# sirpkt/flink-tensorflow

Hardware: AMD Instinct MI355X
Metric: records/sec (whole node) + p50 per-record latency, ResNet-50 stream DP=1/8 (higher is better)
Workload: dtype bf16

## Files before the change

### flink_tensorflow_amd/config.py

```python
from __future__ import annotations

import argparse
import contextlib
import dataclasses
import os
from dataclasses import dataclass, field
from typing import Any

_HBM_BYTES_MI355X = 288 * 1024 ** 3


@dataclass
class EngineConfig:
    parallelism: int = 1
    max_batch: int = 256
    max_delay_ms: float = 10.0
    precision: str = "bf16"
    batch_buckets: tuple = (64, 256)
    arena_fraction: float = 0.9
    use_hip_graph: bool = True
    pipeline_depth: int = 3
    checkpoint_interval_s: float | None = None
    checkpoint_dir: str | None = None
    restart_attempts: int = 0
    restart_delay_s: float = 0.0
    channel_capacity: int = 1024
    log_level: str = "INFO"
    sibling_conv_fusion: bool = True
    fuse_preprocess_stem: bool = True
    fuse_block_tails: bool = True
    decimate_tails: bool = True
    recompute_tails: bool = True
    chain_max_links: int = 2
    pw_res_kernel: bool = True
    conv3x3c64_kernel: bool = True
    chain_batch: int = -1
    chain_min_hw: int = 5041
    chain_edge: bool = True
    wd_fused_step: bool = True
    wd_sparse_exchange: str = "owner"
    wd_bucket_slack: float = 2.0
    jpeg_decode: str = "host"
    extra: dict = field(default_factory=dict)

    @classmethod
    def field_names(cls) -> list[str]:
        return [f.name for f in dataclasses.fields(cls) if f.name != "extra"]

    def _coerce(self, name: str, value: Any) -> Any:
        cur = getattr(self, name)
        typ = {f.name: f.type for f in dataclasses.fields(self)}[name]
        if value is None:
            return None
        if isinstance(value, str):
            if "tuple" in str(typ):
                return tuple(int(v) for v in value.replace(" ", "").split(",") if v)
            if "bool" in str(typ):
                return value.lower() in ("1", "true", "yes", "on")
            if "int" in str(typ) and "float" not in str(typ):
                return int(value)
            if "float" in str(typ):
                return float(value)
            return value
        if isinstance(cur, tuple) and isinstance(value, (list, tuple)):
            return tuple(value)
        return value

    def update(self, values: dict) -> "EngineConfig":
        for k, v in values.items():
            if k in self.field_names():
                setattr(self, k, self._coerce(k, v))
            else:
                self.extra[k] = v
        self.validate()
        return self

    @classmethod
    def from_yaml(cls, path: str, base: "EngineConfig | None" = None) -> "EngineConfig":
        import yaml

        with open(path) as f:
            data = yaml.safe_load(f) or {}
        return (base or cls()).update(data)

    @classmethod
    def from_env(cls, base: "EngineConfig | None" = None, prefix: str = "FT_", environ=None) -> "EngineConfig":
        environ = os.environ if environ is None else environ
        vals = {}
        for name in cls.field_names():
            key = prefix + name.upper()
            if key in environ:
                vals[name] = environ[key]
        return (base or cls()).update(vals)

    @classmethod
    def add_arguments(cls, ap: argparse.ArgumentParser) -> None:
        for name in cls.field_names():
            ap.add_argument("--" + name.replace("_", "-"), dest=f"cfg_{name}", default=None)
        ap.add_argument("--config", dest="cfg_yaml", default=None, help="YAML engine config")

    @classmethod
    def load(cls, argv: list[str] | None = None, environ=None) -> "EngineConfig":
        ap = argparse.ArgumentParser(add_help=False)
        cls.add_arguments(ap)
        ns, _ = ap.parse_known_args(argv if argv is not None else [])
        environ = os.environ if environ is None else environ
        cfg = cls()
        yml = ns.cfg_yaml or environ.get("FT_CONFIG")
        if yml:
            cfg = cls.from_yaml(yml, cfg)
        cfg = cls.from_env(cfg, environ=environ)
        cli = {n: getattr(ns, f"cfg_{n}") for n in cls.field_names() if getattr(ns, f"cfg_{n}") is not None}
        return cfg.update(cli)

    def validate(self) -> None:
        if self.parallelism < 1:
            raise ValueError("parallelism must be >= 1")
        if self.max_batch < 1 or self.max_delay_ms < 0:
# ... 73 lines not shown
```

### flink_tensorflow_amd/graph/conv_lowering.py

```python
from __future__ import annotations

from dataclasses import dataclass

import numpy as np
import torch

from ..ops import fp8 as F8
from ..ops import kernels as K
from ..types.names import TensorName
from .graph import Node
from .ops_nn import same_pads
from .plan import CompileError, Val, _cfg, _coff, _eff_scale, _root, _target, _view

_ACTS = {"Relu": K.ACT_RELU, "Relu6": K.ACT_RELU6, "Sigmoid": K.ACT_SIGMOID, "Tanh": K.ACT_TANH}

LITE_FP8_CFG = 11
_PP_MIN_K = 512

_PLAIN_ACTS = (K.ACT_NONE, K.ACT_RELU)
_DW_ACTS = {"Relu": K.ACT_RELU, "Relu6": K.ACT_RELU6}


@dataclass(frozen=True)
class ConvSite:
# ... 217 lines not shown
            w = w * scale
        w_dev = self._dev(w.reshape(KH * KW, C).contiguous(), torch.bfloat16)
        b_dev = self._dev(bias, torch.float32) if bias is not None else None
        self.params += [w_dev] + ([b_dev] if b_dev is not None else [])
        xin = self._as_bf16(x, node.name)
        out = self._new((N, Ho, Wo, C))
        for a in absorbed:
            self._fused.add(a.name)

        def run(xin=xin, out=out, w_dev=w_dev, b_dev=b_dev):
            K.dwconv2d_nhwc(xin.buf, w_dev, b_dev, stride, pads, dil, act, out=_target(out),
                            out_channel_offset=_coff(out), kernel=(KH, KW))

        self._emit(node.name, "dwconv", run, [xin], [out], {"impl": K.dwconv_impl(KH, KW, stride, dil)})
        self._finish_conv(last, absorbed, out)

    def _prepare_conv(self, node, x, w, bias, residual, act, last, absorbed, stride, pads, dil, out_hw,
                      cout_logical: int | None = None) -> _ConvJob:
        KH, KW, Cin, Cout = w.shape
        padded = cout_logical is not None and cout_logical != Cout
        N, H, W, C = x.shape
        s2d = self._s2d_ok(x, node, C, *stride, *dil, pads[0], pads[2], H, W)
        if s2d:
            w_ohwi, pads = K.s2d_stem_weights(w, H, W, pads)
            x.pre_cfg["s2d"] = True
            x.buf_shape = (N, (H + 1) // 2, (W + 1) // 2, 16)
            x.phys_c = 16
            stride = (1, 1)
            cin_pad = 16
        else:
            phys = x.phys_c or C
            cin_pad = -(-phys // 8) * 8
            w_ohwi = w.permute(3, 0, 1, 2).contiguous()
            if cin_pad != Cin:
                w_ohwi = torch.nn.functional.pad(w_ohwi, (0, cin_pad - Cin))
        w_dev = self._dev(w_ohwi, torch.bfloat16)
        b_dev = self._dev(bias, torch.float32) if bias is not None else None
        self.params += [w_dev] + ([b_dev] if b_dev is not None else [])
        out = self._new((N, *out_hw, cout_logical if padded else Cout), phys_c=Cout if padded else None)
        kernel = tuple(w_ohwi.shape[1:3])
        if (not padded and self.precision == "fp8" and residual is None and act in _PLAIN_ACTS and Cout % 16 == 0
                and self._fp8_consumers_ok(last.name) and self._qscale(last.name) is not None
                and _dconv_ok(self.device.type == "cuda", cin_pad, kernel, stride, dil, 2, False, act)):
            out = self._new((N, *out_hw, Cout), torch.uint8)
            out.qscale = self._qscale(last.name)
        res_val = add_node = None
        if residual is not None:
            add_node, ri = residual
            res_val = self.vals[add_node.inputs[ri]]
        xin = x if s2d else self._ensure_padded(x, cin_pad, node.name)
        for a in absorbed:
            self._fused.add(a.name)
        cfg = _cfg()
        site = ConvSite(
            on_gpu=self.device.type == "cuda", x_shape=tuple(xin.shape), cin=Cin, cin_phys=xin.phys_c or Cin, cout=Cout,
            kernel=kernel, stride=tuple(stride), pads=tuple(pads), dil=tuple(dil), act=act,
            residual=res_val is not None,
            res_plain=(res_val is not None and res_val.qscale is None and res_val.concat_slot is None
                       and tuple(res_val.shape) == tuple(out.shape)),
            res_alias=res_val is not None and res_val.alias_of is not None,
            x_dtype=xin.dtype, out_dtype=out.dtype, out_fp8=out.qscale is not None, out_coff=_coff(out), s2d=s2d,
            conv3x3c64_kernel=cfg.conv3x3c64_kernel, pw_res_kernel=cfg.pw_res_kernel)
        return _ConvJob(node, site, x, xin, out, res_val, add_node, w_ohwi, bias, w_dev, b_dev, last, absorbed)

    def _zero_bias(self, c: _ConvJob) -> torch.Tensor:
        return c.b_dev if c.b_dev is not None else self._dev(torch.zeros(c.site.cout), torch.float32)

    def _emit_dconv(self, c: _ConvJob):
        s, out = c.site, c.out
        Cout, conv_out = s.cout, tuple(c.out.shape)
        bn = 64 if Cout >= 64 else 32
        w_arr = self._dev(K.dconv_bf16_weight_bytes(c.w_ohwi, bn))
        b_dev = c.b_dev if c.b_dev is not None else torch.zeros(Cout, dtype=torch.float32, device=self.device)
        self.params += [w_arr, b_dev]
        pool = self._fusable_maxpool(c.last, s.act, out)
        mpad = None
        if pool is not None:
            pnode, mpad, (Hp, Wp) = pool
            out = self._new((conv_out[0], Hp, Wp, Cout))
            self._fused.add(pnode.name)
        elif self._fold_preprocess(c, w_arr, b_dev, bn):
            return

        def run_d(xin=c.xin, out=out, w_arr=w_arr, b_dev=b_dev, bn=bn, mpad=mpad):
            K.conv2d_direct(xin.buf, w_arr, s.kernel, Cout, b_dev, s.stride, s.pads, s.act,
                            out=_target(out), out_channel_offset=_coff(out), bn=bn,
                            out_scale=_eff_scale(out) if out.qscale is not None else None, maxpool_pad=mpad)

        self._emit(c.node.name, "conv", run_d, [c.xin], [out], {"conv_out": conv_out} if pool else None)
        if pool is not None:
            self.vals[(pool[0].name, 0)] = out
            self.stats["fused_pools"] += 1
            return
        self._finish_conv(c.last, c.absorbed, out)

    def _fold_preprocess(self, c: _ConvJob, w_arr, b_dev, bn) -> bool:
        s, x, out = c.site, c.x, c.out
        pp = x.pre_params
        if not (s.s2d and pp is not None and not pp["resize"]
                and _cfg().fuse_preprocess_stem and len(self.steps) == 1 and self.steps[0].kind == "preprocess"
                and self.steps[0].outputs[0] is x and _root(out) is out and _coff(out) == 0):
            return False
        self.steps.pop()
        xu = pp["x"]
        osc = _eff_scale(out) if out.qscale is not None else None

        def run_u(x=xu, out=out, w_arr=w_arr, b_dev=b_dev, bn=bn, osc=osc, mean=pp["mean"], std=pp["std"],
                  pads=s.pads):
            K.conv2d_direct_u8s2d(x.buf, w_arr, s.kernel, s.cout, b_dev, pads, s.act, mean, std, out=out.buf,
                                  bn=bn, out_scale=osc)

        self._emit(c.node.name, "preprocess", run_u, [xu], [out],
                   {"impl": "dconv_u8s2d", "conv_out": tuple(out.shape)})
        self.stats["fused_preprocess"] = 1
        self._finish_conv(c.last, c.absorbed, out)
        return True

    def _emit_conv3x3c64(self, c: _ConvJob):
        bz, act = self._zero_bias(c), c.site.act

        def run_c(xin=c.xin, out=c.out, w_dev=c.w_dev, bz=bz):
            K.conv3x3_c64(xin.buf, w_dev, bz, act, out=_target(out), out_channel_offset=_coff(out))

        self._emit(c.node.name, "conv", run_c, [c.xin], [c.out], {"impl": "conv3x3c64"})
        self.stats["conv3x3c64"] += 1
        self._finish_conv(c.last, c.absorbed, c.out)

    def _emit_gemm_pp(self, c: _ConvJob):
        Cin, Cout = c.site.cin, c.site.cout
        w_nk = c.w_dev.reshape(Cout, Cin)
        bz = self._zero_bias(c)
        M = int(np.prod(c.xin.shape[:-1]))
        splits = K.gemm_pp_splits(M, Cout, Cin)
        ws = torch.empty(splits * M * Cout, dtype=torch.float32, device=self.device) if splits > 1 else None

        def run_pp(xin=c.xin, out=c.out, w_nk=w_nk, bz=bz, act=c.site.act, splits=splits, ws=ws):
            K.gemm_pp(xin.buf.view(-1, Cin), w_nk, bz, None, act, out=_target(out), out_col=_coff(out),
                      splits=splits, ws=ws)

        self._emit(c.node.name, "gemm", run_pp, [c.xin], [c.out], {"impl": "gemm_pp"})
        self._finish_conv(c.last, c.absorbed, c.out)

    def _emit_pw_res(self, c: _ConvJob):
        w_nk = c.w_dev.reshape(c.site.cout, c.site.cin)
        bz = self._zero_bias(c)

        def run_pw(xin=c.xin, out=c.out, res_val=c.res_val, w_nk=w_nk, bz=bz):
            K.pw_res(xin.buf, w_nk, bz, res_val.buf, out=_target(out), out_channel_offset=_coff(out))

        self._emit(c.node.name, "conv", run_pw, [c.xin, c.res_val], [c.out], {"impl": "pw_res"})
        self.stats["pw_res"] += 1
        self._finish_conv(c.last, c.absorbed, c.out)

    def _emit_conv_lite(self, c: _ConvJob):
        s = c.site
        cl = K.ConvPP([(tuple(c.xin.shape), s.kernel, s.stride, (s.pads[0], s.pads[2]), s.dil)], s.cout,
                      tuple(c.out.shape[1:3]), self.device)

        def run_l(xin=c.xin, out=c.out, res_val=c.res_val, cl=cl, w2=c.w_dev.reshape(s.cout, -1), b_dev=c.b_dev):
            cl([xin.buf], w2, b_dev, res_val.buf if res_val is not None else None, s.act, out=_target(out),
               out_channel_offset=_coff(out))

        self.stats["conv_lite"] += 1
        self._emit_single_conv(c, run_l)

    def _emit_igemm(self, c: _ConvJob):
        s = c.site

        def run(xin=c.xin, out=c.out, res_val=c.res_val, w_dev=c.w_dev, b_dev=c.b_dev):
            K.conv2d_nhwc(xin.buf, w_dev, b_dev, res_val.buf if res_val is not None else None, s.stride,
# ... 544 lines not shown
```

### flink_tensorflow_amd/kernels/dconv.hip

```cpp
#include <pybind11/pybind11.h>

#include <stdexcept>
#include <string>

#include "common.h"

typedef int i32x8 __attribute__((ext_vector_type(8)));

namespace {

__device__ __attribute__((aligned(16))) uint32_t g_zero16[4];

constexpr int TH = 16, TW = 16;

struct DconvParams {
  const uint8_t* x;
  const uint8_t* w;
  const float* scale;
  const float* bias;
  uint8_t* y;
  float out_q;
  int N, H, W, Cin, Ho, Wo, Cout, KH, KW, S, ph, pw;
  int RB;
  int WP;
// ... 162 lines not shown
    } else {
      i32x8 a[I], bb[J];
#pragma unroll
      for (int i = 0; i < I; ++i) {
        const uint8_t* src = Wsm + (i * 16 + frow) * p.WP + kb;
        const u32x4 lo = *reinterpret_cast<const u32x4*>(src), hi = *reinterpret_cast<const u32x4*>(src + 16);
        a[i] = i32x8{(int)lo[0], (int)lo[1], (int)lo[2], (int)lo[3], (int)hi[0], (int)hi[1], (int)hi[2], (int)hi[3]};
      }
#pragma unroll
      for (int j = 0; j < J; ++j) {
        const uint8_t* src = Ps + prow0[j] * p.RB + bo;
        const u32x4 lo = *reinterpret_cast<const u32x4*>(src), hi = *reinterpret_cast<const u32x4*>(src + 16);
        bb[j] = i32x8{(int)lo[0], (int)lo[1], (int)lo[2], (int)lo[3], (int)hi[0], (int)hi[1], (int)hi[2], (int)hi[3]};
      }
#pragma unroll
      for (int i = 0; i < I; ++i)
#pragma unroll
        for (int j = 0; j < J; ++j)
          acc[i][j] = __builtin_amdgcn_mfma_scale_f32_16x16x128_f8f6f4(a[i], bb[j], acc[i][j], 0, 0, 0, 127, 0, 127);
    }
  }
  FTM_PRIO_LO(p.prio);
  __syncthreads();

  uint8_t* Os = smem;
#pragma unroll
  for (int i = 0; i < I; ++i) {
    const int cl = i * 16 + fq * 4;
    f32x4 sv = {1.f, 1.f, 1.f, 1.f}, bv = {0.f, 0.f, 0.f, 0.f};
    if (n0 + cl < p.Cout) {
      if constexpr (ES == 1) sv = *reinterpret_cast<const f32x4*>(p.scale + n0 + cl);
      bv = *reinterpret_cast<const f32x4*>(p.bias + n0 + cl);
    }
#pragma unroll
    for (int j = 0; j < J; ++j) {
      const int pl = (wave * J + j) * TW + frow;
      float v[4];
#pragma unroll
      for (int r = 0; r < 4; ++r) v[r] = apply_act<ACT>(acc[i][j][r] * sv[r] + bv[r]);
      if constexpr (POOL) {
        const int oy = oy0 + pl / TPW, ox = ox0 + pl % TPW;
        if ((unsigned)oy >= (unsigned)p.Ho || (unsigned)ox >= (unsigned)p.Wo) v[0] = v[1] = v[2] = v[3] = 0.f;
      }
      if constexpr (OUT_FP8) {
        *reinterpret_cast<uint32_t*>(Os + pl * OLD + cl) =
            pack4_fp8(v[0] * p.out_q, v[1] * p.out_q, v[2] * p.out_q, v[3] * p.out_q);
      } else {
        bf16x4 o;
        o[0] = f2bf(v[0]); o[1] = f2bf(v[1]); o[2] = f2bf(v[2]); o[3] = f2bf(v[3]);
        *reinterpret_cast<bf16x4*>(Os + pl * OLD + cl * 2) = o;
      }
    }
  }
  __syncthreads();
  constexpr int EPO = 16 / OB;
  constexpr int CPR = BN / EPO;
  if constexpr (POOL) {
    for (int q = tid; q < PTH * 8 * CPR; q += NTH) {
      const int pp = q / CPR, cc = q % CPR;
      const int pyl = pp >> 3, pxl = pp & 7;
      const int py = (oy0 + p.ppt) / 2 + pyl, px = (ox0 + p.ppl) / 2 + pxl;
      const int c = n0 + cc * EPO;
      if (py >= p.Hp || px >= p.Wp || c >= p.Cout) continue;
      const uint8_t* src = Os + ((2 * pyl) * TPW + 2 * pxl) * OLD + cc * 16;
      const size_t mo = ((size_t)n * p.Hp + py) * p.Wp + px;
      if constexpr (OUT_FP8)
        *reinterpret_cast<u8x16*>(p.y + mo * p.ldy + p.y_coff + c) = pool3x3_max_u8(src, TPW * OLD, OLD);
      else
        *reinterpret_cast<u16x8*>(p.y + (mo * p.ldy + p.y_coff + c) * 2) = pool3x3_max(src, TPW * OLD, OLD);
    }
    return;
  }
  for (int q = tid; q < THE * TW * CPR; q += NTH) {
    const int pl = q / CPR, cc = q % CPR;
    const int oy = oy0 + pl / TW, ox = ox0 + pl % TW;
    const int c = n0 + cc * EPO;
    if (oy >= p.Ho || ox >= p.Wo || c >= p.Cout) continue;
    const u32x4 v = *reinterpret_cast<const u32x4*>(Os + pl * OLD + cc * 16);
    const size_t m = ((size_t)n * p.Ho + oy) * p.Wo + ox;
    *reinterpret_cast<u32x4*>(p.y + (m * p.ldy + p.y_coff + c) * OB) = v;
  }
}

template <int ES, int BN, bool OUT_FP8, int WAVES>
void launch_act(const DconvParams& p, int act, size_t lds, hipStream_t s) {
  dim3 grid(p.N * p.tiles_h * p.tiles_w * p.tiles_n), block(WAVES * 64);
  if constexpr ((ES == 2 && !OUT_FP8) || (ES == 1 && OUT_FP8)) {
    if (p.Hp > 0) {
      if (act != ACT_RELU) throw std::invalid_argument("dconv: fused pool needs a ReLU conv");
      static bool done = false;
      if (!done) {
        hipFuncSetAttribute((const void*)dconv_kernel<ES, BN, ACT_RELU, OUT_FP8, true, WAVES>,
                            hipFuncAttributeMaxDynamicSharedMemorySize, 160 * 1024);
        done = true;
      }
      hipLaunchKernelGGL((dconv_kernel<ES, BN, ACT_RELU, OUT_FP8, true, WAVES>), grid, block, lds, s, p);
      return;
    }
  } else {
    if (p.Hp > 0) throw std::invalid_argument("dconv: fused pool needs bf16 -> bf16 or fp8 -> fp8");
  }
  switch (act) {
    case ACT_NONE:
      hipLaunchKernelGGL((dconv_kernel<ES, BN, ACT_NONE, OUT_FP8, false, WAVES>), grid, block, lds, s, p);
      break;
    case ACT_RELU:
      hipLaunchKernelGGL((dconv_kernel<ES, BN, ACT_RELU, OUT_FP8, false, WAVES>), grid, block, lds, s, p);
      break;
    default: throw std::invalid_argument("dconv: activation must be none/relu");
  }
}

template <int BN, bool OUT_FP8, int WAVES>
void launch_u8(const DconvParams& p, int act, size_t lds, hipStream_t s) {
  dim3 grid(p.N * p.tiles_h * p.tiles_w * p.tiles_n), block(WAVES * 64);
  static bool done = false;
  if (!done) {
    for (auto f : {(const void*)dconv_kernel<2, BN, ACT_NONE, OUT_FP8, false, WAVES, true>,
                   (const void*)dconv_kernel<2, BN, ACT_RELU, OUT_FP8, false, WAVES, true>})
      hipFuncSetAttribute(f, hipFuncAttributeMaxDynamicSharedMemorySize, 160 * 1024);
    done = true;
  }
  if (act == ACT_RELU) hipLaunchKernelGGL((dconv_kernel<2, BN, ACT_RELU, OUT_FP8, false, WAVES, true>), grid, block, lds, s, p);
  else if (act == ACT_NONE) hipLaunchKernelGGL((dconv_kernel<2, BN, ACT_NONE, OUT_FP8, false, WAVES, true>), grid, block, lds, s, p);
  else throw std::invalid_argument("dconv: activation must be none/relu");
}

template <int ES, int BN, bool OUT_FP8, int WAVES>
void set_lds_limit() {
  static bool done = false;
  if (done) return;
  for (auto f : {(const void*)dconv_kernel<ES, BN, ACT_NONE, OUT_FP8, false, WAVES>,
                 (const void*)dconv_kernel<ES, BN, ACT_RELU, OUT_FP8, false, WAVES>})
    hipFuncSetAttribute(f, hipFuncAttributeMaxDynamicSharedMemorySize, 160 * 1024);
  done = true;
}

}

int patch_rows(int KH, int S, bool pool, int npx) { return (pool ? (npx - 1) / 17 : npx / TW - 1) * S + KH; }

int lds_bytes(int es, int bn, int KH, int KW, int S, int Cin, int wp, bool pool, int npx = TH * TW) {
  const int PH = patch_rows(KH, S, pool, npx), PW = (pool ? TW : TW - 1) * S + KW;
  const int patch = PH * PW * Cin * es;
  const int ob = 2;
  int need = ((patch + 1023) & ~1023) + bn * wp + 1024;
  const int epi = npx * (bn * ob + 16);
  return need > epi ? need : epi;
}

void dconv(uintptr_t x, uintptr_t w, uintptr_t scale, uintptr_t bias, uintptr_t y, int es, int N, int H, int W,
           int Cin, int Cout, int KH, int KW, int S, int ph, int pw, int Ho, int Wo, int wp, int ldy, int y_coff,
           int out_fp8, float out_q, int act, int bn, uintptr_t stream, int Hp, int Wp, int ppt, int ppl,
           int waves) {
  const int KL = es == 2 ? 16 : 32;
  if (es != 1 && es != 2) throw std::invalid_argument("dconv: es must be 1 or 2");
  if ((Cin * es) % KL) throw std::invalid_argument("dconv: Cin*es must be a multiple of " + std::to_string(KL));
  if (bn != 32 && bn != 64) throw std::invalid_argument("dconv: bn must be 32 or 64");
  const int kb = KH * KW * Cin * es;
  const int kpad = (kb + 4 * KL - 1) / (4 * KL) * (4 * KL);
  if (wp != kpad + 16) throw std::invalid_argument("dconv: weight pitch must be round_up(K bytes, 4*KL) + 16");
  const int oe = out_fp8 ? 16 : 8;
  if (Cout % oe || ldy % oe || y_coff % oe) throw std::invalid_argument("dconv: Cout/ldy/y_coff alignment");
  if (S != 1 && S != 2) throw std::invalid_argument("dconv: stride must be 1 or 2");
  if (!bias || (es == 1 && !scale)) throw std::invalid_argument("dconv: bias (and fp8 scale) required");
  if (x % 16 || w % 16 || y % 16 || bias % 16 || (scale && scale % 16)) throw std::invalid_argument("dconv: alignment");
  if (waves != 4 && waves != 8) throw std::invalid_argument("dconv: waves must be 4 or 8");
  if (waves == 8 && lds_bytes(es, bn, KH, KW, S, Cin, wp, Hp > 0, 512) > 160 * 1024) waves = 4;
  const int npx = waves * 64;
  const int pool_rows = waves == 8 ? 14 : 7;
  const int lds = lds_bytes(es, bn, KH, KW, S, Cin, wp, Hp > 0, npx);
  if (lds > 160 * 1024) throw std::invalid_argument("dconv: tile does not fit LDS (" + std::to_string(lds) + " B)");
  DconvParams p{};
  p.x = reinterpret_cast<const uint8_t*>(x);
  p.w = reinterpret_cast<const uint8_t*>(w);
  p.scale = reinterpret_cast<const float*>(scale);
  p.bias = reinterpret_cast<const float*>(bias);
  p.y = reinterpret_cast<uint8_t*>(y);
  p.out_q = out_q;
  p.N = N; p.H = H; p.W = W; p.Cin = Cin; p.Ho = Ho; p.Wo = Wo; p.Cout = Cout; p.KH = KH; p.KW = KW; p.S = S;
  p.ph = ph; p.pw = pw;
  p.RB = Cin * es;
  p.WP = wp;
  p.ksteps = kpad / (4 * KL);
  if (p.ksteps > 64) throw std::invalid_argument("dconv: more than 64 K-steps");
  p.PH = patch_rows(KH, S, Hp > 0, npx);
  p.PW = (Hp > 0 ? TW : TW - 1) * S + KW;
  p.ldy = ldy; p.y_coff = y_coff;
  p.prio = ftm_mfma_prio();
  p.Hp = Hp; p.Wp = Wp; p.ppt = ppt; p.ppl = ppl;
  for (int st = 0; st < p.ksteps; ++st)
    for (int fq = 0; fq < 4; ++fq) {
      const int kb = st * 4 * KL + fq * KL;
      int tap = kb / p.RB;
      const int cb = kb - tap * p.RB;
      if (tap >= KH * KW) tap = 0;
      const int dy = tap / KW, dx = tap - dy * KW;
      p.koff[st * 4 + fq] = (dy * p.PW + dx) * p.RB + cb;
    }
  if (Hp > 0) {
    if (ppt < 0 || ppt > 1 || ppl < 0 || ppl > 1) throw std::invalid_argument("dconv: pool padding must be 0/1");
    if ((Hp - 1) * 2 + 3 > Ho + ppt + 1 || (Wp - 1) * 2 + 3 > Wo + ppl + 1)
      throw std::invalid_argument("dconv: pooled shape inconsistent with conv output");
    p.tiles_h = (Hp + pool_rows - 1) / pool_rows;
    p.tiles_w = (Wp + 7) / 8;
  } else {
    p.tiles_h = (Ho + npx / TW - 1) / (npx / TW);
    p.tiles_w = (Wo + TW - 1) / TW;
  }
  p.tiles_n = (Cout + bn - 1) / bn;
  hipStream_t s = reinterpret_cast<hipStream_t>(stream);
#define FTM_DCONV(ES_, BN_, OF_)                                                   \
  do {                                                                             \
    if (waves == 8) {                                                              \
      set_lds_limit<ES_, BN_, OF_, 8>();                                           \
      launch_act<ES_, BN_, OF_, 8>(p, act, lds, s);                                \
    } else {                                                                       \
      set_lds_limit<ES_, BN_, OF_, 4>();                                           \
      launch_act<ES_, BN_, OF_, 4>(p, act, lds, s);                                \
    }                                                                              \
  } while (0)
  if (es == 2) {
    if (bn == 32) { if (out_fp8) FTM_DCONV(2, 32, true); else FTM_DCONV(2, 32, false); }
    else { if (out_fp8) FTM_DCONV(2, 64, true); else FTM_DCONV(2, 64, false); }
  } else {
    if (bn == 32) { if (out_fp8) FTM_DCONV(1, 32, true); else FTM_DCONV(1, 32, false); }
    else { if (out_fp8) FTM_DCONV(1, 64, true); else FTM_DCONV(1, 64, false); }
  }
#undef FTM_DCONV
  FTM_CHECK_LAUNCH();
}

void dconv_u8s2d(uintptr_t x, uintptr_t w, uintptr_t bias, uintptr_t y, int N, int Hi, int Wi, int Cout, int KH, int KW,
                 int ph, int pw, int Ho, int Wo, int wp, int ldy, int y_coff, int out_fp8, float out_q, int act, int bn,
                 float m0, float m1, float m2, float s0, float s1, float s2, uintptr_t stream, int waves) {
  const int Cin = 16, es = 2, KL = 16;
  if (bn != 32 && bn != 64) throw std::invalid_argument("dconv_u8s2d: bn must be 32 or 64");
  const int kb = KH * KW * Cin * es;
  const int kpad = (kb + 4 * KL - 1) / (4 * KL) * (4 * KL);
  if (wp != kpad + 16) throw std::invalid_argument("dconv_u8s2d: weight pitch must be round_up(K bytes, 64) + 16");
  const int oe = out_fp8 ? 16 : 8;
  if (Cout % oe || ldy % oe || y_coff % oe) throw std::invalid_argument("dconv_u8s2d: Cout/ldy/y_coff alignment");
  if (!bias || w % 16 || y % 16 || bias % 16) throw std::invalid_argument("dconv_u8s2d: bias / alignment");
  if (waves != 4 && waves != 8) throw std::invalid_argument("dconv_u8s2d: waves must be 4 or 8");
  if (waves == 8 && lds_bytes(es, bn, KH, KW, 1, Cin, wp, false, 512) > 160 * 1024) waves = 4;
  const int npx = waves * 64;
  const int lds = lds_bytes(es, bn, KH, KW, 1, Cin, wp, false, npx);
  if (lds > 160 * 1024) throw std::invalid_argument("dconv_u8s2d: tile does not fit LDS");
  DconvParams p{};
  p.x = nullptr;
  p.xu8 = reinterpret_cast<const uint8_t*>(x);
  p.Hi = Hi; p.Wi = Wi;
  p.mean[0] = m0; p.mean[1] = m1; p.mean[2] = m2;
  p.istd[0] = s0; p.istd[1] = s1; p.istd[2] = s2;
  p.w = reinterpret_cast<const uint8_t*>(w);
  p.scale = nullptr;
  p.bias = reinterpret_cast<const float*>(bias);
  p.y = reinterpret_cast<uint8_t*>(y);
  p.out_q = out_q;
  p.N = N; p.H = (Hi + 1) / 2; p.W = (Wi + 1) / 2; p.Cin = Cin; p.Ho = Ho; p.Wo = Wo; p.Cout = Cout;
  p.KH = KH; p.KW = KW; p.S = 1; p.ph = ph; p.pw = pw;
  p.RB = Cin * es;
  p.WP = wp;
  p.ksteps = kpad / (4 * KL);
  if (p.ksteps > 64) throw std::invalid_argument("dconv_u8s2d: more than 64 K-steps");
  p.PH = patch_rows(KH, 1, false, npx);
  p.PW = (TW - 1) + KW;
  p.ldy = ldy; p.y_coff = y_coff;
  p.prio = ftm_mfma_prio();
  for (int st = 0; st < p.ksteps; ++st)
    for (int fq = 0; fq < 4; ++fq) {
      const int kb2 = st * 4 * KL + fq * KL;
      int tap = kb2 / p.RB;
      const int cb = kb2 - tap * p.RB;
      if (tap >= KH * KW) tap = 0;
      const int dy = tap / KW, dx = tap - dy * KW;
      p.koff[st * 4 + fq] = (dy * p.PW + dx) * p.RB + cb;
    }
  p.tiles_h = (Ho + npx / TW - 1) / (npx / TW);
  p.tiles_w = (Wo + TW - 1) / TW;
  p.tiles_n = (Cout + bn - 1) / bn;
  hipStream_t s = reinterpret_cast<hipStream_t>(stream);
#define FTM_U8(BN_, OF_)                                              \
  do {                                                                \
    if (waves == 8) launch_u8<BN_, OF_, 8>(p, act, lds, s);            \
    else launch_u8<BN_, OF_, 4>(p, act, lds, s);                       \
  } while (0)
  if (bn == 32) { if (out_fp8) FTM_U8(32, true); else FTM_U8(32, false); }
  else { if (out_fp8) FTM_U8(64, true); else FTM_U8(64, false); }
#undef FTM_U8
  FTM_CHECK_LAUNCH();
}

void register_dconv(pybind11::module_& m) {
  m.def("dconv", &dconv);
  m.def("dconv_u8s2d", &dconv_u8s2d);
}
```

### flink_tensorflow_amd/ops/kernels.py

```python
from __future__ import annotations

import copy
import functools
import os

import torch
import torch.nn.functional as F

from .. import _ext

ACT_NONE, ACT_RELU, ACT_GELU, ACT_SIGMOID, ACT_TANH, ACT_RELU6, ACT_DRELU = 0, 1, 2, 3, 4, 5, 6
_ACT_NAMES = {None: ACT_NONE, "none": ACT_NONE, "relu": ACT_RELU, "gelu": ACT_GELU, "gelu_tanh": ACT_GELU,
              "sigmoid": ACT_SIGMOID, "tanh": ACT_TANH, "relu6": ACT_RELU6, "drelu": ACT_DRELU}


def act_code(act) -> int:
    if isinstance(act, int):
        return act
    try:
        return _ACT_NAMES[act]
    except KeyError:
        raise ValueError(f"unknown activation {act!r}") from None


# ... 1059 lines not shown

def embed_layernorm(ids: torch.Tensor, type_ids: torch.Tensor | None, word: torch.Tensor, pos: torch.Tensor,
                    type_emb: torch.Tensor, gamma: torch.Tensor, beta: torch.Tensor, seq: int, eps: float = 1e-12,
                    out: torch.Tensor | None = None, pos_ids: torch.Tensor | None = None) -> torch.Tensor:
    T = ids.numel()
    V, D = word.shape
    if out is None:
        out = torch.empty((T, D), dtype=word.dtype, device=word.device)
    if ids.is_cuda:
        _check(ids, "ids", torch.int32, ids.device)
        for t, n in ((word, "word"), (pos, "pos"), (type_emb, "type"), (out, "out")):
            _check(t, n, device=ids.device)
        if type_ids is not None:
            _check(type_ids, "type_ids", torch.int32, ids.device)
        if pos_ids is not None:
            _check(pos_ids, "pos_ids", torch.int32, ids.device)
        if pos.shape[0] < seq:
            raise ValueError("embed_layernorm: position table shorter than the sequence")
        _hip().embed_ln_bf16(ids.data_ptr(), _ptr(type_ids), _ptr(pos_ids), word.data_ptr(), pos.data_ptr(),
                             type_emb.data_ptr(), gamma.data_ptr(), beta.data_ptr(), out.data_ptr(), T, seq, D, V,
                             float(eps), _stream())
        return out
    idx = ids.long().clamp(0, V - 1)
    p = pos_ids.long() if pos_ids is not None else torch.arange(T) % seq
    x = word.float()[idx] + pos.float()[p]
    x = x + type_emb.float()[type_ids.long() if type_ids is not None else torch.zeros(T, dtype=torch.long)]
    out.copy_(F.layer_norm(x, (D,), gamma.float(), beta.float(), eps).to(out.dtype))
    return out


def layernorm(x: torch.Tensor, gamma: torch.Tensor, beta: torch.Tensor, residual: torch.Tensor | None = None,
              eps: float = 1e-12, out=None, sum_out=None) -> torch.Tensor:
    D = x.shape[-1]
    rows = x.numel() // D
    if out is None:
        out = torch.empty_like(x)
    if x.is_cuda:
        _check(x, "x", device=x.device)
        _check(out, "out", device=x.device)
        _check(gamma, "gamma", torch.float32, x.device)
        _check(beta, "beta", torch.float32, x.device)
        if residual is not None:
            _check(residual, "residual", device=x.device)
        _hip().layernorm_bf16(x.data_ptr(), _ptr(residual), gamma.data_ptr(), beta.data_ptr(), out.data_ptr(),
                              _ptr(sum_out), rows, D, float(eps), _stream())
        return out
    s = x.float() + (residual.float() if residual is not None else 0)
    if sum_out is not None:
        sum_out.copy_(s.to(sum_out.dtype))
    out.copy_(F.layer_norm(s, (D,), gamma.float(), beta.float(), eps).to(out.dtype))
    return out


def dconv_eligible(Cin: int, KH: int, KW: int, stride, dilation, es: int, bn: int = 64) -> bool:
    sh, sw = stride
    if sh != sw or sh not in (1, 2) or tuple(dilation) != (1, 1) or KH * KW == 1:
        return False
    kl = 16 if es == 2 else 32
    if (Cin * es) % kl:
        return False
    kb = KH * KW * Cin * es
    wp = -(-kb // (4 * kl)) * (4 * kl) + 16
    ph, pw = 15 * sh + KH, 15 * sw + KW
    lds = ((ph * pw * Cin * es + 1023) & ~1023) + bn * wp + 1024
    return lds <= 96 * 1024


def dconv_weights(w_ohwi_bytes: torch.Tensor, Cout: int, es: int, bn: int) -> torch.Tensor:
    kl = 16 if es == 2 else 32
    kb = w_ohwi_bytes.shape[1]
    wp = -(-kb // (4 * kl)) * (4 * kl) + 16
    cpad = -(-Cout // bn) * bn
    out = torch.zeros((cpad, wp), dtype=torch.uint8, device=w_ohwi_bytes.device)
    out[:Cout, :kb] = w_ohwi_bytes
    return out


def dconv_bf16_weight_bytes(w_ohwi: torch.Tensor, bn: int) -> torch.Tensor:
    Cout = w_ohwi.shape[0]
    wb = w_ohwi.to(torch.bfloat16).contiguous().reshape(Cout, -1).view(torch.uint8)
    return dconv_weights(wb, Cout, 2, bn)


def _dconv_waves(waves, pool_rows, bn) -> int:
    if waves is None and pool_rows is not None:
        waves = {7: 4, 14: 8}[int(pool_rows)]
    return int(waves or (8 if bn == 64 else 4))


def conv2d_direct(x: torch.Tensor, w_arr: torch.Tensor, kshape, Cout: int, bias: torch.Tensor, stride=(1, 1),
                  pad=(0, 0, 0, 0), act=None, out: torch.Tensor | None = None, out_channel_offset: int = 0,
                  bn: int = 64, chan_scale: torch.Tensor | None = None, out_scale: float | None = None,
                  maxpool_pad: tuple | None = None, pool_rows: int | None = None,
                  waves: int | None = None) -> torch.Tensor:
    N, H, W, Cin = x.shape
    KH, KW = kshape
    s = stride[0]
    pt, pb, pl, pr = pad
    Ho, Wo = conv_out_hw(H, W, KH, KW, s, s, pt, pl, 1, 1, pb, pr)
    es = 2 if x.dtype == torch.bfloat16 else 1
    out_fp8 = out_scale is not None
    Hp = Wp = ppt = ppl = 0
    oh, ow = Ho, Wo
    if maxpool_pad is not None:
        ppt, ppb, ppl, ppr = maxpool_pad
        Hp, Wp = (Ho + ppt + ppb - 3) // 2 + 1, (Wo + ppl + ppr - 3) // 2 + 1
        oh, ow = Hp, Wp
    if out is None:
        out = torch.empty((N, oh, ow, Cout), dtype=torch.uint8 if out_fp8 else torch.bfloat16, device=x.device)
        out_channel_offset = 0
    if out.shape[:3] != (N, oh, ow) or out_channel_offset + Cout > out.shape[3]:
        raise ValueError(f"conv2d_direct: out {tuple(out.shape)} cannot hold [{N},{oh},{ow},{Cout}]")
    if es == 1 and chan_scale is None:
        raise ValueError("conv2d_direct: fp8 input needs chan_scale")
    _check(x, "x", x.dtype, x.device)
    _check(w_arr, "w", torch.uint8, x.device)
    _check(bias, "bias", torch.float32, x.device)
    _check(out, "out", torch.uint8 if out_fp8 else torch.bfloat16, x.device)
    _hip().dconv(x.data_ptr(), w_arr.data_ptr(), _ptr(chan_scale), bias.data_ptr(), out.data_ptr(), es, N, H, W, Cin,
                 Cout, KH, KW, s, pt, pl, Ho, Wo, w_arr.shape[1], out.shape[3], out_channel_offset, int(out_fp8),
                 1.0 / out_scale if out_fp8 else 1.0, act_code(act), bn, _stream(), Hp, Wp, ppt, ppl,
                 _dconv_waves(waves, pool_rows, bn))
    return out


def conv2d_direct_u8s2d(x_u8: torch.Tensor, w_arr: torch.Tensor, kshape, Cout: int, bias: torch.Tensor, pad, act,
                        mean, std, out: torch.Tensor | None = None, bn: int = 64, out_scale: float | None = None,
                        waves: int | None = None) -> torch.Tensor:
    N, Hi, Wi, _ = x_u8.shape
    KH, KW = kshape
    pt, pb, pl, pr = pad
    Hb, Wb = (Hi + 1) // 2, (Wi + 1) // 2
    Ho, Wo = conv_out_hw(Hb, Wb, KH, KW, 1, 1, pt, pl, 1, 1, pb, pr)
    out_fp8 = out_scale is not None
    if out is None:
        out = torch.empty((N, Ho, Wo, Cout), dtype=torch.uint8 if out_fp8 else torch.bfloat16, device=x_u8.device)
    if tuple(out.shape[:3]) != (N, Ho, Wo) or out.shape[3] < Cout:
        raise ValueError(f"conv2d_direct_u8s2d: out {tuple(out.shape)} cannot hold [{N},{Ho},{Wo},{Cout}]")
    _check(x_u8, "x", torch.uint8, x_u8.device)
    _check(w_arr, "w", torch.uint8, x_u8.device)
    _check(bias, "bias", torch.float32, x_u8.device)
    _check(out, "out", torch.uint8 if out_fp8 else torch.bfloat16, x_u8.device)
    _hip().dconv_u8s2d(x_u8.data_ptr(), w_arr.data_ptr(), bias.data_ptr(), out.data_ptr(), N, Hi, Wi, Cout, KH, KW, pt,
                       pl, Ho, Wo, w_arr.shape[1], out.shape[3], 0, int(out_fp8), 1.0 / out_scale if out_fp8 else 1.0,
                       act_code(act), bn, float(mean[0]), float(mean[1]), float(mean[2]), 1.0 / std[0], 1.0 / std[1],
                       1.0 / std[2], _stream(), _dconv_waves(waves, None, bn))
    return out


def conv1x1_dual(x: torch.Tensor, x2: torch.Tensor, w_cat: torch.Tensor, bias: torch.Tensor, stride2: int = 1,
                 act=None, out: torch.Tensor | None = None, out_channel_offset: int = 0, cfg: int = -1) -> torch.Tensor:
    N, Ho, Wo, K1 = x.shape
    _, H2, W2, C2 = x2.shape
    Cout = w_cat.shape[0]
    if w_cat.shape[1] != K1 + C2:
        raise ValueError(f"conv1x1_dual: weights K {w_cat.shape[1]} != {K1} + {C2}")
    if out is None:
        out = torch.empty((N, Ho, Wo, Cout), dtype=x.dtype if x.is_cuda else torch.float32, device=x.device)
        out_channel_offset = 0
    if x2.shape[0] != N or (Ho - 1) * stride2 >= H2 or (Wo - 1) * stride2 >= W2:
        raise ValueError(f"conv1x1_dual: shortcut source {tuple(x2.shape)} at stride {stride2} does not cover "
                         f"[{N},{Ho},{Wo}]")
    if out.shape[:3] != (N, Ho, Wo) or out_channel_offset + Cout > out.shape[3]:
        raise ValueError(f"conv1x1_dual: out {tuple(out.shape)} cannot hold [{N},{Ho},{Wo},{Cout}] at "
                         f"offset {out_channel_offset}")
    a = act_code(act)
    if x.is_cuda:
        for t, n in ((x, "x"), (x2, "x2"), (w_cat, "w"), (out, "out")):
            _check(t, n, device=x.device)
        _check(bias, "bias", torch.float32, x.device)
        _hip().conv1x1_dual_bf16(x.data_ptr(), x2.data_ptr(), w_cat.data_ptr(), bias.data_ptr(), out.data_ptr(), N, Ho,
                                 Wo, K1, C2, H2, W2, stride2, Cout, out.shape[3], out_channel_offset, a, _stream(), cfg)
        return out
    xs = x2[:, ::stride2, ::stride2, :][:, :Ho, :Wo, :]
    y = x.float() @ w_cat[:, :K1].float().t() + xs.float() @ w_cat[:, K1:].float().t() + bias.float()
    out[..., out_channel_offset:out_channel_offset + Cout] = _apply_act_ref(y, a).to(out.dtype)
    return out


def pw_res_ok(K_: int, N: int, num_cu: int = 256) -> bool:
    return K_ in (128, 256) and N % 128 == 0 and 8 * (N // 128) <= num_cu


def pw_res(x: torch.Tensor, w_nk: torch.Tensor, bias: torch.Tensor, residual: torch.Tensor,
           out: torch.Tensor | None = None, out_channel_offset: int = 0, tp: int = 0) -> torch.Tensor:
    K_ = x.shape[-1]
    N = w_nk.shape[0]
    lead = tuple(x.shape[:-1])
    if not pw_res_ok(K_, N) or tuple(w_nk.reshape(N, -1).shape) != (N, K_):
        raise ValueError(f"pw_res: unsupported shapes x {tuple(x.shape)}, w {tuple(w_nk.shape)}")
    if tuple(residual.shape) != (*lead, N) or bias.numel() != N:
        raise ValueError("pw_res: residual must be [..., N] and bias [N]")
    if out is None:
        out = torch.empty((*lead, N), dtype=x.dtype if x.is_cuda else torch.float32, device=x.device)
        out_channel_offset = 0
    if tuple(out.shape[:-1]) != lead or out_channel_offset + N > out.shape[-1]:
        raise ValueError(f"pw_res: out {tuple(out.shape)} cannot hold [..., {N}] at offset {out_channel_offset}")
    M = x.numel() // K_
    if x.is_cuda:
        for t, n in ((x, "x"), (w_nk, "w"), (residual, "residual"), (out, "out")):
            _check(t, n, device=x.device)
        _check(bias, "bias", torch.float32, x.device)
        dev = x.device.index if x.device.index is not None else torch.cuda.current_device()
        _hip().pw_res_bf16(x.data_ptr(), w_nk.data_ptr(), bias.data_ptr(), residual.data_ptr(), out.data_ptr(), M, N,
                           K_, out.shape[-1], out_channel_offset, residual.shape[-1], _NUM_CU[dev], _stream(), tp)
# ... 74 lines not shown
```

Baseline: 82230.

## Add specialized bf16 stem conv+maxpool kernel with MFMA and LDS tiling

Adds a dedicated HIP kernel for the ResNet-50 stem convolution: the 4x4 space-to-depth conv with ReLU and fused 3x3/2 maxpool, in bf16. Weights and the input patch are DMA'd into LDS. The kernel runs a double-buffered MFMA 16x16x32 loop, stages the output tile in LDS and pools from there. It is dispatched when shape conditions match and a new config flag (default on) allows it. The aim is to beat the generic direct-conv kernel on this layer, at the cost of a large hand-tuned kernel with rigid shape assumptions and a high LDS budget.

```diff
diff --git a/flink_tensorflow_amd/config.py b/flink_tensorflow_amd/config.py
--- a/flink_tensorflow_amd/config.py
+++ b/flink_tensorflow_amd/config.py
@@ -34,6 +34,7 @@
     chain_max_links: int = 2
     pw_res_kernel: bool = True
     conv3x3c64_kernel: bool = True
+    stem_kernel: bool = True
     chain_batch: int = -1
     chain_min_hw: int = 5041
     chain_edge: bool = True
diff --git a/flink_tensorflow_amd/graph/conv_lowering.py b/flink_tensorflow_amd/graph/conv_lowering.py
--- a/flink_tensorflow_amd/graph/conv_lowering.py
+++ b/flink_tensorflow_amd/graph/conv_lowering.py
@@ -323,10 +323,11 @@
         elif self._fold_preprocess(c, w_arr, b_dev, bn):
             return
 
-        def run_d(xin=c.xin, out=out, w_arr=w_arr, b_dev=b_dev, bn=bn, mpad=mpad):
+        def run_d(xin=c.xin, out=out, w_arr=w_arr, b_dev=b_dev, bn=bn, mpad=mpad, generic=not _cfg().stem_kernel):
             K.conv2d_direct(xin.buf, w_arr, s.kernel, Cout, b_dev, s.stride, s.pads, s.act,
                             out=_target(out), out_channel_offset=_coff(out), bn=bn,
-                            out_scale=_eff_scale(out) if out.qscale is not None else None, maxpool_pad=mpad)
+                            out_scale=_eff_scale(out) if out.qscale is not None else None, maxpool_pad=mpad,
+                            generic_stem=generic)
 
         self._emit(c.node.name, "conv", run_d, [c.xin], [out], {"conv_out": conv_out} if pool else None)
         if pool is not None:
diff --git a/flink_tensorflow_amd/kernels/dconv.hip b/flink_tensorflow_amd/kernels/dconv.hip
--- a/flink_tensorflow_amd/kernels/dconv.hip
+++ b/flink_tensorflow_amd/kernels/dconv.hip
@@ -268,6 +268,158 @@
   }
 }
 
+namespace stem {
+constexpr int RB = 32, KT = 4, CW = 17, NPX = 512, NTH = 512, BN = 64, PTH = 14, KS = 8;
+constexpr int PW = TW + KT, PH = (NPX - 1) / CW + KT;
+constexpr int WP = KT * KT * RB + 16;
+constexpr int PCH = PH * PW * RB / 16, WCH = BN * WP / 16;
+constexpr int WOFF = (PH * PW * RB + 1023) & ~1023;
+constexpr int OLD = BN * 2 + 16, BOFF = NPX * OLD, LDS = BOFF + BN * 4;
+static_assert(WCH % 64 == 0 && (PCH + 63) / 64 * 1024 <= WOFF, "DMA wave-instructions stay inside their regions");
+static_assert(WOFF + BN * WP <= BOFF, "the bias row lies behind patch, bank and output tile");
+static_assert(KS * 64 + 16 == WP && PTH * 8 * (BN / 8) <= 2 * NTH, "K-steps / pooled items");
+}
+
+typedef float f32x2 __attribute__((ext_vector_type(2)));
+typedef __bf16 bf16x2 __attribute__((ext_vector_type(2)));
+
+FTM_DEVICE uint32_t pack2_bf16(float lo, float hi) {
+  return __builtin_bit_cast(uint32_t, __builtin_convertvector(f32x2{lo, hi}, bf16x2));
+}
+
+__global__ __launch_bounds__(stem::NTH) __attribute__((amdgpu_waves_per_eu(4))) void dconv_stem_kernel(DconvParams p) {
+  using namespace stem;
+  extern __shared__ __attribute__((aligned(16))) uint8_t smem[];
+  int b = blockIdx.x;
+  const int tn = b % p.tiles_n; b /= p.tiles_n;
+  const int tw = b % p.tiles_w; b /= p.tiles_w;
+  const int th = b % p.tiles_h;
+  const int n = b / p.tiles_h;
+  const int oy0 = th * (2 * PTH) - p.ppt, ox0 = tw * 16 - p.ppl, n0 = tn * BN;
+  const int tid = threadIdx.x, lane = tid & 63, wave = tid >> 6;
+  uint8_t* Ps = smem;
+  uint8_t* Wsm = smem + WOFF;
+  float* Bs = reinterpret_cast<float*>(smem + BOFF);
+
+  {
+    const uint8_t* wb = p.w + (size_t)n0 * WP;
+#pragma unroll
+    for (int it = 0; it < (WCH + NTH - 1) / NTH; ++it) {
+      const int q0 = wave * 64 + it * NTH;
+      if (q0 < WCH) glds16(wb + (size_t)(q0 + lane) * 16, Wsm + q0 * 16);
+    }
+    const uint8_t* xb = p.x + (size_t)n * p.H * p.W * RB;
+    const unsigned r0 = tid >> 1, py0 = r0 / PW;
+    int iy = oy0 - p.ph + (int)py0, ix = ox0 - p.pw + (int)(r0 - py0 * PW);
+    const int ix_wrap = ox0 - p.pw + PW;
+#pragma unroll
+    for (int it = 0; it < (PCH + NTH - 1) / NTH; ++it) {
+      const int q0 = wave * 64 + it * NTH;
+      if (q0 < PCH) {
+        const bool ok = (unsigned)iy < (unsigned)p.H && (unsigned)ix < (unsigned)p.W;
+        const void* src = ok ? (const void*)(xb + ((unsigned)(iy * p.W + ix) * RB + (lane & 1) * 16)) : (const void*)g_zero16;
+        glds16(src, Ps + q0 * 16);
+      }
+      iy += NTH / 2 / PW, ix += NTH / 2 % PW;
+      if (ix >= ix_wrap) ix -= PW, ++iy;
+    }
+  }
+  const float bias_l = n0 + lane < p.Cout ? p.bias[n0 + lane] : 0.f;
+  const int frow = lane & 15, fq = lane >> 4;
+  const uint8_t* Ab = Wsm + frow * WP + fq * 16;
+  const uint8_t* Bb[4];
+  unsigned live = 0;
+#pragma unroll
+  for (int j = 0; j < 4; ++j) {
+    const unsigned pix = (wave * 4 + j) * 16 + frow, r = pix / CW, c = pix - r * CW;
+    Bb[j] = Ps + (r * PW + c) * RB + fq * 16;
+    if ((unsigned)(oy0 + (int)r) < (unsigned)p.Ho && (unsigned)(ox0 + (int)c) < (unsigned)p.Wo) live |= 1u << j;
+  }
+  asm volatile("s_waitcnt vmcnt(0)" ::: "memory");
+  if (wave == 0) Bs[lane] = bias_l;
+  __syncthreads();
+
+  f32x4 acc[4][4];
+#pragma unroll
+  for (int i = 0; i < 4; ++i)
+#pragma unroll
+    for (int j = 0; j < 4; ++j) acc[i][j] = f32x4{0.f, 0.f, 0.f, 0.f};
+  bf16x8 a[4], bb[2][4];
+  auto read_a = [&](int i, int s) { a[i] = *reinterpret_cast<const bf16x8*>(Ab + i * 16 * WP + s * 64); };
+  auto read_b = [&](int s, bf16x8(&dst)[4]) {
+#pragma unroll
+    for (int j = 0; j < 4; ++j) dst[j] = *reinterpret_cast<const bf16x8*>(Bb[j] + ((s >> 1) * PW + (s & 1) * 2) * RB);
+  };
+  read_b(0, bb[0]);
+#pragma unroll
+  for (int i = 0; i < 4; ++i) read_a(i, 0);
+#pragma unroll
+  for (int s = 0; s < KS; ++s) {
+    if (s + 1 < KS) read_b(s + 1, bb[(s + 1) & 1]);
+    __builtin_amdgcn_sched_barrier(0);
+#pragma unroll
+    for (int i = 0; i < 4; ++i) {
+#pragma unroll
+      for (int j = 0; j < 4; ++j) acc[i][j] = __builtin_amdgcn_mfma_f32_16x16x32_bf16(a[i], bb[s & 1][j], acc[i][j], 0, 0, 0);
+      __builtin_amdgcn_sched_barrier(0);
+      if (s + 1 < KS) read_a(i, s + 1);
+      __builtin_amdgcn_sched_barrier(0);
+    }
+  }
+  uint32_t o[4][4][2];
+#pragma unroll
+  for (int i = 0; i < 4; ++i) {
+    const f32x4 bv = *reinterpret_cast<const f32x4*>(Bs + i * 16 + fq * 4);
+#pragma unroll
+    for (int j = 0; j < 4; ++j) {
+      const uint32_t keep = 0u - ((live >> j) & 1u);
+      float v[4];
+#pragma unroll
+      for (int r = 0; r < 4; ++r) v[r] = apply_act<ACT_RELU>(acc[i][j][r] + bv[r]);
+      o[i][j][0] = pack2_bf16(v[0], v[1]) & keep;
+      o[i][j][1] = pack2_bf16(v[2], v[3]) & keep;
+    }
+  }
+  __syncthreads();
+  uint8_t* Os = smem;
+#pragma unroll
+  for (int i = 0; i < 4; ++i)
+#pragma unroll
+    for (int j = 0; j < 4; ++j) {
+      const int pl = (wave * 4 + j) * 16 + frow;
+      *reinterpret_cast<uint2*>(Os + pl * OLD + (i * 16 + fq * 4) * 2) = uint2{o[i][j][0], o[i][j][1]};
+    }
+  __syncthreads();
+#pragma unroll
+  for (int it = 0; it < 2; ++it) {
+    const int q = tid + it * NTH;
+    const int pp = q >> 3, cc = q & 7;
+    const int pyl = pp >> 3, pxl = pp & 7;
+    const int py = th * PTH + pyl, px = tw * 8 + pxl;
+    const int c = n0 + cc * 8;
+    if (q >= PTH * 8 * 8 || py >= p.Hp || px >= p.Wp || c >= p.Cout) continue;
+    const uint8_t* src = Os + ((2 * pyl) * CW + 2 * pxl) * OLD + cc * 16;
+    const size_t mo = ((size_t)n * p.Hp + py) * p.Wp + px;
+    *reinterpret_cast<u16x8*>(p.y + (mo * p.ldy + p.y_coff + c) * 2) = pool3x3_max(src, CW * OLD, OLD);
+  }
+}
+
+bool stem_config(const DconvParams& p, int es, int bn, int out_fp8, int act, int waves) {
+  return es == 2 && bn == stem::BN && !out_fp8 && act == ACT_RELU && p.Hp > 0 && waves == 8 && p.Cin == 16 &&
+         p.KH == stem::KT && p.KW == stem::KT && p.S == 1 && p.WP == stem::WP &&
+         (long long)p.H * p.W * stem::RB < (1LL << 31);
+}
+
+void launch_stem(const DconvParams& p, hipStream_t s) {
+  static bool done = false;
+  if (!done) {
+    (void)hipFuncSetAttribute((const void*)dconv_stem_kernel, hipFuncAttributeMaxDynamicSharedMemorySize, 160 * 1024);
+    done = true;
+  }
+  dim3 grid(p.N * p.tiles_h * p.tiles_w * p.tiles_n), block(stem::NTH);
+  hipLaunchKernelGGL(dconv_stem_kernel, grid, block, stem::LDS, s, p);
+}
+
 template <int ES, int BN, bool OUT_FP8, int WAVES>
 void launch_act(const DconvParams& p, int act, size_t lds, hipStream_t s) {
   dim3 grid(p.N * p.tiles_h * p.tiles_w * p.tiles_n), block(WAVES * 64);
@@ -335,10 +487,10 @@
   return need > epi ? need : epi;
 }
 
-void dconv(uintptr_t x, uintptr_t w, uintptr_t scale, uintptr_t bias, uintptr_t y, int es, int N, int H, int W,
-           int Cin, int Cout, int KH, int KW, int S, int ph, int pw, int Ho, int Wo, int wp, int ldy, int y_coff,
-           int out_fp8, float out_q, int act, int bn, uintptr_t stream, int Hp, int Wp, int ppt, int ppl,
-           int waves) {
+const char* dconv(uintptr_t x, uintptr_t w, uintptr_t scale, uintptr_t bias, uintptr_t y, int es, int N, int H, int W,
+                  int Cin, int Cout, int KH, int KW, int S, int ph, int pw, int Ho, int Wo, int wp, int ldy, int y_coff,
+                  int out_fp8, float out_q, int act, int bn, uintptr_t stream, int Hp, int Wp, int ppt, int ppl,
+                  int waves, int generic_stem) {
   const int KL = es == 2 ? 16 : 32;
   if (es != 1 && es != 2) throw std::invalid_argument("dconv: es must be 1 or 2");
   if ((Cin * es) % KL) throw std::invalid_argument("dconv: Cin*es must be a multiple of " + std::to_string(KL));
@@ -396,6 +548,11 @@
   }
   p.tiles_n = (Cout + bn - 1) / bn;
   hipStream_t s = reinterpret_cast<hipStream_t>(stream);
+  if (!generic_stem && stem_config(p, es, bn, out_fp8, act, waves)) {
+    launch_stem(p, s);
+    FTM_CHECK_LAUNCH();
+    return "dconv_stem";
+  }
 #define FTM_DCONV(ES_, BN_, OF_)                                                   \
   do {                                                                             \
     if (waves == 8) {                                                              \
@@ -415,6 +572,7 @@
   }
 #undef FTM_DCONV
   FTM_CHECK_LAUNCH();
+  return "dconv";
 }
 
 void dconv_u8s2d(uintptr_t x, uintptr_t w, uintptr_t bias, uintptr_t y, int N, int Hi, int Wi, int Cout, int KH, int KW,
diff --git a/flink_tensorflow_amd/ops/kernels.py b/flink_tensorflow_amd/ops/kernels.py
--- a/flink_tensorflow_amd/ops/kernels.py
+++ b/flink_tensorflow_amd/ops/kernels.py
@@ -1165,6 +1165,9 @@
     return dconv_weights(wb, Cout, 2, bn)
 
 
+last_dconv_kernel: str | None = None
+
+
 def _dconv_waves(waves, pool_rows, bn) -> int:
     if waves is None and pool_rows is not None:
         waves = {7: 4, 14: 8}[int(pool_rows)]
@@ -1175,7 +1178,8 @@
                   pad=(0, 0, 0, 0), act=None, out: torch.Tensor | None = None, out_channel_offset: int = 0,
                   bn: int = 64, chan_scale: torch.Tensor | None = None, out_scale: float | None = None,
                   maxpool_pad: tuple | None = None, pool_rows: int | None = None,
-                  waves: int | None = None) -> torch.Tensor:
+                  waves: int | None = None, generic_stem: bool = False) -> torch.Tensor:
+    global last_dconv_kernel
     N, H, W, Cin = x.shape
     KH, KW = kshape
     s = stride[0]
@@ -1200,10 +1204,11 @@
     _check(w_arr, "w", torch.uint8, x.device)
     _check(bias, "bias", torch.float32, x.device)
     _check(out, "out", torch.uint8 if out_fp8 else torch.bfloat16, x.device)
-    _hip().dconv(x.data_ptr(), w_arr.data_ptr(), _ptr(chan_scale), bias.data_ptr(), out.data_ptr(), es, N, H, W, Cin,
-                 Cout, KH, KW, s, pt, pl, Ho, Wo, w_arr.shape[1], out.shape[3], out_channel_offset, int(out_fp8),
-                 1.0 / out_scale if out_fp8 else 1.0, act_code(act), bn, _stream(), Hp, Wp, ppt, ppl,
-                 _dconv_waves(waves, pool_rows, bn))
+    last_dconv_kernel = _hip().dconv(
+        x.data_ptr(), w_arr.data_ptr(), _ptr(chan_scale), bias.data_ptr(), out.data_ptr(), es, N, H, W, Cin,
+        Cout, KH, KW, s, pt, pl, Ho, Wo, w_arr.shape[1], out.shape[3], out_channel_offset, int(out_fp8),
+        1.0 / out_scale if out_fp8 else 1.0, act_code(act), bn, _stream(), Hp, Wp, ppt, ppl,
+        _dconv_waves(waves, pool_rows, bn), int(generic_stem))
     return out
 
 
```

New measurement: 83200 (median of 4 runs). About the same (+1.2%).
